# dusk-network/plonk_gadgets

Hardware: AMD Instinct MI355X
Metric: gadget constraints/sec (range_check 256-bit) (higher is better)
Workload: dtype u64x4 (BLS12-381 scalar, Montgomery limbs); 1 GPU; C2: 2^20 witnesses/GPU x (allocate + range_check(min=0,max=2^254)), n=255, 1031 rows + 1034 vars per witness; items_per_gpu=1048576, items_per_launch=1048576

## Files before the change

### plonk_gadgets_amd/csrc/capi.hip

```cpp
#include "../../include/plonk_gadgets_hip.h"

#include <hip/hip_runtime.h>

#include <algorithm>
#include <cstdio>
#include <cstdlib>
#include <cstring>
#include <initializer_list>
#include <new>
#include <functional>
#include <string>
#include <type_traits>
#include <utility>
#include <vector>

#include "emit.hpp"
#include "fr.hpp"
#include "range_gadgets.hpp"
#include "scalar_gadgets.hpp"
#include "composer.hpp"
#include "permutation.hpp"
#include "materialize.hpp"
#include "permutation_product.hpp"
#include "ntt.hpp"
// ... 63 lines not shown
}
pg_status check_u64s(const void *p, const char *what, bool nullable = false) {
    if (!p && nullable) return PG_OK;
    if (!p || !aligned(p, 8)) return fail(PG_ERR_INVALID_ARGUMENT, std::string(what) + " NULL or not 8-byte aligned");
    return PG_OK;
}

}

struct pg_engine {
    int device = -1;
    int num_cus = 0;
    uint4 *d_pow2 = nullptr;
    uint32_t *d_rows = nullptr, *d_vars = nullptr;
    uint64_t *d_blk_rows = nullptr, *d_blk_vars = nullptr;
    unsigned long long *d_blk_agg = nullptr;
    uint32_t *d_err_count = nullptr;
    uint64_t scratch_items = 0, scratch_blocks = 0;
    using PlanResult = pg::PlanTotals;
    PlanResult *h_plan = nullptr;
    uint4 *d_prefix = nullptr;
    uint64_t inv_elems = 0;
    hipStream_t side = nullptr;
    hipEvent_t ev_fork = nullptr, ev_inv = nullptr;
    hipStream_t last_stream = nullptr;
    bool have_last = false;
    hipEvent_t ev_switch = nullptr;
    uint4 *d_pp = nullptr;
    uint64_t pp_units = 0;
    uint4 *d_ntt = nullptr;
    uint64_t ntt_units = 0;
    uint4 *d_quot = nullptr, *d_eval = nullptr;
    uint64_t quot_units = 0, eval_units = 0;
};

namespace {

pg_status ensure_scratch(pg_engine *e, uint64_t batch) {
    if (batch <= e->scratch_items && e->d_err_count) return PG_OK;
    PG_HIP_TRY(hipSetDevice(e->device));
    if (e->d_rows) { (void)hipFree(e->d_rows); e->d_rows = nullptr; }
    if (e->d_vars) { (void)hipFree(e->d_vars); e->d_vars = nullptr; }
    if (e->d_blk_rows) { (void)hipFree(e->d_blk_rows); e->d_blk_rows = nullptr; }
    if (e->d_blk_vars) { (void)hipFree(e->d_blk_vars); e->d_blk_vars = nullptr; }
    if (e->d_blk_agg) { (void)hipFree(e->d_blk_agg); e->d_blk_agg = nullptr; }
    e->scratch_items = 0;
    const uint64_t items = batch < 1024 ? 1024 : batch;
    const uint64_t nblk = std::max<uint64_t>((items + pg::kScanBlock - 1) / pg::kScanBlock, 2048);
    PG_HIP_TRY(hipMalloc(&e->d_rows, items * sizeof(uint32_t)));
    PG_HIP_TRY(hipMalloc(&e->d_vars, items * sizeof(uint32_t)));
    PG_HIP_TRY(hipMalloc(&e->d_blk_rows, nblk * sizeof(uint64_t)));
    PG_HIP_TRY(hipMalloc(&e->d_blk_vars, nblk * sizeof(uint64_t)));
    PG_HIP_TRY(hipMalloc(&e->d_blk_agg, (nblk + 1) * sizeof(unsigned long long)));
    PG_HIP_TRY(hipMemset(e->d_blk_agg, 0, (nblk + 1) * sizeof(unsigned long long)));
    e->scratch_blocks = nblk;
    if (!e->d_err_count) {
        PG_HIP_TRY(hipMalloc(&e->d_err_count, sizeof(uint32_t)));
        PG_HIP_TRY(hipMemset(e->d_err_count, 0, sizeof(uint32_t)));
    }
    e->scratch_items = items;
    return PG_OK;
}

pg::PlanScan plan_scan(pg_engine *e, uint64_t batch, uint64_t *d_row_off, uint64_t *d_var_off, bool with_errs) {
    const uint64_t nblk = (batch + pg::kScanBlock - 1) / pg::kScanBlock;
    pg::PlanScan P{};
// ... 1356 lines not shown
```

### plonk_gadgets_amd/csrc/capi_composer.inc

```

struct pg_composer {
    pg_engine *e = nullptr;
    hipStream_t stream = nullptr;
    uint64_t gate_cap = 0, var_cap = 0, n = 0, nvars = 0, zero_var = 0;
    pg::ComposerCols cols{};
    uint64_t *d_stage = nullptr;
    std::vector<uint64_t> pi_gate;
    std::vector<pg_scalar> pi_val;
    std::vector<pg::FourthWire> fourth;
    std::vector<pg::PermSeg> segs;
    void *perm_small = nullptr, *perm_big = nullptr, *val_ws = nullptr;
    void *perm_pieces = nullptr;
    size_t perm_pieces_bytes = 0;
    size_t perm_small_bytes = 0, perm_big_bytes = 0, val_ws_bytes = 0;
    std::vector<void *> ragged;
    uint64_t *h_total = nullptr;
    uint64_t perm_last_sparse = 0;
    uint64_t sparse_hint = 0;
    uint64_t sparse_cap_first = 0;
    bool auto_grow = false;
    uint64_t col_stride = 0;
    void *block = nullptr;
    struct Queued {
        uint8_t kind;
        pg::GateCmd g;
        pg::Fr b0, b1;
        uint32_t num_bits;
        uint64_t wvar;
        pg::Fr wval;
        uint64_t gate, var;
        bool in_place = false;
    };
    std::vector<Queued> queue;
    bool queueing = true;
    pg_scalar last_min{}, last_max{};
    pg_layout last_lay{};
    int last_kind = 0;
    struct Staging {
        char *h = nullptr, *d = nullptr;
        size_t bytes = 0;
        hipEvent_t ev = nullptr;
    } staging[2];
    int stage = 0;
    size_t queue_used = 0;
    uint64_t flushes = 0, flush_launches = 0;
    struct Sig {
// ... 613 lines not shown
    c->rows_in_place = c->rows_rewritten = 0;
    return PG_OK;
}

pg_status pg_composer_refresh_stats(const pg_composer *c, uint64_t *rows_in_place, uint64_t *rows_rewritten, int *refreshing) {
    if (!c) return fail(PG_ERR_INVALID_ARGUMENT, "composer is NULL");
    if (rows_in_place) *rows_in_place = c->rows_in_place;
    if (rows_rewritten) *rows_rewritten = c->rows_rewritten;
    if (refreshing) *refreshing = c->refill ? 1 : 0;
    return PG_OK;
}

void pg_composer_destroy(pg_composer *c) {
    if (!c) return;
    (void)hipSetDevice(c->e->device);
    (void)hipStreamSynchronize(c->stream);
    if (c->block) {
        (void)hipFree(c->block);
    } else {
        for (int i = 0; i < 5; i++) if (c->cols.q[i]) (void)hipFree(c->cols.q[i]);
        for (int i = 0; i < 3; i++) if (c->cols.w[i]) (void)hipFree(c->cols.w[i]);
        if (c->cols.vars) (void)hipFree(c->cols.vars);
    }
    if (c->d_stage) (void)hipFree(c->d_stage);
    for (pg_composer::Staging &S : c->staging) {
        if (S.d) (void)hipFree(S.d);
        if (S.h) (void)hipHostFree(S.h);
        if (S.ev) (void)hipEventDestroy(S.ev);
    }
    if (c->perm_small) (void)hipFree(c->perm_small);
    if (c->perm_big) (void)hipFree(c->perm_big);
    if (c->val_ws) (void)hipFree(c->val_ws);
    if (c->perm_pieces) (void)hipFree(c->perm_pieces);
    for (void *p : c->ragged) (void)hipFree(p);
    if (c->h_total) (void)hipHostFree(c->h_total);
    delete c;
}

uint64_t pg_composer_circuit_size(const pg_composer *c) { return c ? c->n : 0; }
uint64_t pg_composer_num_variables(const pg_composer *c) { return c ? c->nvars : 0; }
pg_variable pg_composer_zero_var(const pg_composer *c) { return c ? c->zero_var : 0; }

pg_status pg_composer_columns(const pg_composer *c, pg_columns *out) {
    if (!c || !out) return fail(PG_ERR_INVALID_ARGUMENT, "NULL argument");
    PG_TRY(flush(const_cast<pg_composer *>(c)));
    *out = cols_at(c, 0, 0);
    return PG_OK;
}

pg_status pg_composer_reserve(pg_composer *c, uint64_t gate_capacity, uint64_t var_capacity) {
    if (!c) return fail(PG_ERR_INVALID_ARGUMENT, "composer is NULL");
    return grow(c, gate_capacity, var_capacity);
}
pg_status pg_composer_spread_columns(pg_composer *c, uint64_t stride_bytes) {
    if (!c) return fail(PG_ERR_INVALID_ARGUMENT, "composer is NULL");
    if (stride_bytes > (1ull << 44)) return fail(PG_ERR_INVALID_ARGUMENT, "stride too large");
    if (stride_bytes == c->col_stride) return PG_OK;
    const uint64_t before = c->col_stride;
    c->col_stride = stride_bytes;
    const pg_status st = grow(c, c->gate_cap, c->var_cap, true);
    if (st != PG_OK) c->col_stride = before;
    return st;
}
pg_status pg_composer_auto_grow(pg_composer *c, int on) {
    if (!c) return fail(PG_ERR_INVALID_ARGUMENT, "composer is NULL");
    c->auto_grow = on != 0;
// ... 858 lines not shown
        else if (s.wire_kind == pg::WIRES_MAX_BOUND_ALLOCATED) PG_MAT_LAUNCH(pg::MAT_SELF, pg::WIRES_MAX_BOUND_ALLOCATED);
        else if (s.wire_kind == pg::WIRES_DECOMPOSITION) PG_MAT_LAUNCH(pg::MAT_SELF, pg::WIRES_DECOMPOSITION);
        else if (s.wire_kind == pg::WIRES_MIX) PG_MAT_LAUNCH(pg::MAT_SELF, pg::WIRES_MIX);
        else PG_MAT_LAUNCH(pg::MAT_READ_WIRES, pg::WIRES_UNKNOWN);
#undef PG_MAT_LAUNCH
        at = s.gate_end;
    }
    generic(at, c->n);
    CallBuffers B(c->stream);
    uint64_t *d_gate; uint4 *d_val; pg::FourthWire *d_fw;
    PG_TRY(upload_sparse(c, B, &d_gate, &d_val, &d_fw));
    if (d_fw)
        hipLaunchKernelGGL(pg::patch_fourth_kernel, dim3(1), dim3(64), 0, c->stream, reinterpret_cast<uint4 *>(out->q_4), out->w_4,
                           reinterpret_cast<uint4 *>(out->w_4_value), c->cols.vars, d_fw, (uint32_t)c->fourth.size());
    PG_HIP_TRY(hipGetLastError());
    PG_HIP_TRY(hipStreamSynchronize(c->stream));
    return PG_OK;
}

#ifndef PG_PERM_LDS_PAD
#define PG_PERM_LDS_PAD 0
#endif
static pg_status perm_reserve(pg_composer *c, void **buf, size_t *have, size_t bytes) {
    if (bytes <= *have) return PG_OK;
    PG_HIP_TRY(hipStreamSynchronize(c->stream));
    if (*buf) (void)hipFree(*buf);
    *buf = nullptr;
    *have = 0;
    PG_HIP_TRY(hipMalloc(buf, bytes));
    *have = bytes;
    return PG_OK;
}

pg_status pg_composer_permutation_reserve(pg_composer *c, uint64_t sparse_positions) {
    if (!c) return fail(PG_ERR_INVALID_ARGUMENT, "composer is NULL");
    c->sparse_cap_first = sparse_positions;
    if (sparse_positions) c->perm_last_sparse = 0;
    return PG_OK;
}

pg_status pg_composer_permutation(pg_composer *c, uint64_t padded_n, uint64_t *d_sigma) {
    if (!c) return fail(PG_ERR_INVALID_ARGUMENT, "composer is NULL");
    PG_TRY(flush(c));
    PG_TRY(check_u64s(d_sigma, "d_sigma"));
    if (padded_n < c->n) return fail(PG_ERR_INVALID_ARGUMENT, "padded_n is smaller than the circuit");
    PG_HIP_TRY(hipSetDevice(c->e->device));
    const uint32_t grid = (uint32_t)c->e->num_cus * 32;
    if (!c->h_total) PG_HIP_TRY(hipHostMalloc(reinterpret_cast<void **>(&c->h_total), 32, hipHostMallocDefault));
    uint32_t pos_bits = 2, var_bits = 1;
    while ((1ull << pos_bits) < 4 * c->n) pos_bits++;
    while ((1ull << var_bits) < c->nvars + 1) var_bits++;
    if (pos_bits + var_bits > 64) return fail(PG_ERR_INVALID_ARGUMENT, "circuit too large for 64-bit (Variable, position) keys");
    std::vector<pg::PermSeg> segs;
    std::vector<std::pair<uint64_t, uint64_t>> gaps;
    uint64_t at = 0, gap_rows = 0;
    for (pg::PermSeg s : c->segs) {
        const auto fits = [&](uint64_t k) {
            return 4 * k * s.L < pg::kPermDone && k * s.V < pg::kPermNone &&
                   pg::perm_local_lds_bytes((uint32_t)(k * s.L), (uint32_t)(k * s.V)) <= pg::kPermLocalLdsLimit;
        };
        if (!fits(1)) continue;
        uint64_t k = 1024 / s.L;
        k = k < 1 ? 1 : (k > s.items ? s.items : k);
        while (k > 1 && !fits(k)) k--;
        const bool closed_ladder = s.wire_kind != pg::WIRES_UNKNOWN && s.wire_kind < pg::WIRES_MIX && (s.row_off ? s.wire_kind == pg::WIRES_MAX_BOUND && s.tail == 0 : s.wire_n >= 2);
        if (closed_ladder || (pg::is_template_kind(s.wire_kind) && s.tail == 0)) k = 1;
        s.group = (uint32_t)k;
        if (s.gate_base > at) gaps.emplace_back(at, s.gate_base);
        segs.push_back(s);
        at = s.gate_end;
    }
    if (c->n > at) gaps.emplace_back(at, c->n);
    for (const auto &g : gaps) gap_rows += g.second - g.first;
    const size_t seg_bytes = (segs.size() * sizeof(pg::PermSeg) + 255) / 256 * 256;
    const size_t fw_bytes = (c->fourth.size() * sizeof(pg::FourthWire) + 255) / 256 * 256;
    PG_TRY(perm_reserve(c, &c->perm_small, &c->perm_small_bytes, seg_bytes + fw_bytes + 256));
    char *small = static_cast<char *>(c->perm_small);
    pg::PermCtx X;
    X.C = c->cols; X.n = c->n; X.padded_n = padded_n; X.zero_var = c->zero_var;
    X.segs = reinterpret_cast<const pg::PermSeg *>(small); X.n_segs = (uint32_t)segs.size();
    X.fw = reinterpret_cast<const pg::FourthWire *>(small + seg_bytes); X.n_fw = (uint32_t)c->fourth.size();
    X.fw_lo = 0; X.fw_span = 0; X.pos_bits = pos_bits;
    X.hole_key = pos_bits + var_bits >= 64 ? ~0ull : (1ull << (pos_bits + var_bits)) - 1;
    if (!c->fourth.empty()) {
        uint64_t lo = ~0ull, hi = 0;
        for (const pg::FourthWire &f : c->fourth) { lo = f.gate < lo ? f.gate : lo; hi = f.gate > hi ? f.gate : hi; }
        X.fw_lo = lo; X.fw_span = hi - lo;
    }
    uint64_t reserved = 0;
    for (pg::PermSeg &s : segs)
        if (s.wire_kind != pg::WIRES_UNKNOWN && !s.row_off && s.wire_n >= 2) {
            s.sparse_base = reserved;
            reserved += s.items * pg::ladder_foreign_per_item(s.wire_kind);
        } else if (pg::is_template_kind(s.wire_kind) && s.tail == 0) {
            s.sparse_base = reserved;
            reserved += s.items * pg::template_foreign_per_item(s.wire_kind);
        }
    const auto ragged_ladder = [](const pg::PermSeg &s) { return s.row_off && s.wire_kind == pg::WIRES_MAX_BOUND && s.tail == 0; };
    const auto template_seg = [](const pg::PermSeg &s) { return pg::is_template_kind(s.wire_kind) && s.tail == 0; };
    const auto needs_pieces = [&](const pg::PermSeg &s) { return ragged_ladder(s) || (template_seg(s) && s.row_off); };
    const auto pieces_of = [](const pg::PermSeg &s) { return (s.gate_end - (s.gate_base & ~1ull) + pg::kPermLadderRows - 1) / pg::kPermLadderRows; };
    {
        uint64_t total_pieces = 0;
        for (const pg::PermSeg &s : segs)
            if (needs_pieces(s)) total_pieces += pieces_of(s);
        if (total_pieces) {
            PG_TRY(perm_reserve(c, &c->perm_pieces, &c->perm_pieces_bytes, total_pieces * sizeof(uint32_t)));
            uint32_t *at_piece = static_cast<uint32_t *>(c->perm_pieces);
            for (pg::PermSeg &s : segs)
                if (needs_pieces(s)) {
                    s.piece_item = at_piece;
                    at_piece += pieces_of(s);
                    const uint64_t want = (s.items + pg::kThreads - 1) / pg::kThreads;
                    hipLaunchKernelGGL(pg::perm_piece_items_kernel, dim3((uint32_t)(want < grid ? want : grid)), dim3(pg::kThreads), 0, c->stream, s,
                                       pg::kPermLadderRows, at_piece - pieces_of(s));
                }
            PG_HIP_TRY(hipGetLastError());
        }
    }
    unsigned long long *d_count = reinterpret_cast<unsigned long long *>(small + seg_bytes + fw_bytes);
    if (!segs.empty())
        PG_HIP_TRY(hipMemcpyAsync(small, segs.data(), segs.size() * sizeof(pg::PermSeg), hipMemcpyHostToDevice, c->stream));
    if (!c->fourth.empty())
        PG_HIP_TRY(hipMemcpyAsync(small + seg_bytes, c->fourth.data(), c->fourth.size() * sizeof(pg::FourthWire),
                                  hipMemcpyHostToDevice, c->stream));
    uint64_t cap = c->sparse_cap_first ? c->sparse_cap_first : 4 * gap_rows + c->sparse_hint + (1ull << 16), nS = 0;
    if (cap < c->perm_last_sparse) cap = c->perm_last_sparse;
    uint64_t *k0 = nullptr, *k1 = nullptr, holes = 0;
    size_t tmp_bytes = 0;
    for (int attempt = 0;; attempt++) {
        uint64_t *nul = nullptr;
        PG_HIP_TRY(rocprim::radix_sort_keys(nullptr, tmp_bytes, nul, nul, (size_t)cap, 0u, pos_bits + var_bits, c->stream));
        const size_t kb = (cap * 8 + 255) / 256 * 256;
        PG_TRY(perm_reserve(c, &c->perm_big, &c->perm_big_bytes, 2 * kb + tmp_bytes + 256));
        k0 = reinterpret_cast<uint64_t *>(c->perm_big);
        k1 = reinterpret_cast<uint64_t *>(static_cast<char *>(c->perm_big) + kb);
        const pg::PermSparse Q{k0, d_count, cap};
        hipLaunchKernelGGL(pg::perm_count_init_kernel, dim3(1), dim3(1), 0, c->stream, d_count, reserved);
        for (const pg::PermSeg &s : segs) {
            const uint64_t groups = (s.items + s.group - 1) / s.group, most = (uint64_t)c->e->num_cus * 64;
            if (s.wire_kind != pg::WIRES_UNKNOWN && !s.row_off && s.wire_n >= 2) {
                const uint64_t pieces = (s.gate_end - (s.gate_base & ~1ull) + pg::kPermLadderRows - 1) / pg::kPermLadderRows;
                const uint64_t lmost = pg::kPermLadderRows <= 2048 ? 0x7fffffffull : most;
                if (pg::kPermLadderLds)
                    PG_HIP_TRY(hipFuncSetAttribute(reinterpret_cast<const void *>(pg::perm_ladder_kernel<false>), hipFuncAttributeMaxDynamicSharedMemorySize,
                                                   (int)pg::kPermLadderLds));
                const uint32_t lds = pg::ladder_foreign_per_item(s.wire_kind) ? 0u : pg::kPermLadderLds;
                hipLaunchKernelGGL(pg::perm_ladder_kernel<false>, dim3((uint32_t)(pieces < lmost ? pieces : lmost)), dim3(pg::kThreads), lds,
                                   c->stream, X, s, Q, d_sigma);
                continue;
            }
            if (template_seg(s)) {
                const uint64_t pieces = pieces_of(s);
                if (pieces > 0x7fffffffull) return fail(PG_ERR_INVALID_ARGUMENT, "segment too large for one launch");
                const uint32_t lds = pg::template_foreign_per_item(s.wire_kind) ? 0u : pg::kPermLadderLds - 8192;
                const pg::TemplateRows T = pg::template_rows(s.wire_kind);
                if (s.row_off) {
                    PG_HIP_TRY(hipFuncSetAttribute(reinterpret_cast<const void *>(pg::perm_template_kernel<true>),
                                                   hipFuncAttributeMaxDynamicSharedMemorySize, (int)pg::kPermLadderLds));
                    hipLaunchKernelGGL(pg::perm_template_kernel<true>, dim3((uint32_t)pieces), dim3(pg::kThreads), lds, c->stream, X, s, T, Q, d_sigma);
                } else {
                    PG_HIP_TRY(hipFuncSetAttribute(reinterpret_cast<const void *>(pg::perm_template_kernel<false>),
                                                   hipFuncAttributeMaxDynamicSharedMemorySize, (int)pg::kPermLadderLds));
                    hipLaunchKernelGGL(pg::perm_template_kernel<false>, dim3((uint32_t)pieces), dim3(pg::kThreads), lds, c->stream, X, s, T, Q, d_sigma);
                }
                continue;
            }
            if (ragged_ladder(s)) {
                const uint64_t pieces = pieces_of(s);
                if (pieces > 0x7fffffffull) return fail(PG_ERR_INVALID_ARGUMENT, "segment too large for one launch");
                if (pg::kPermLadderLds)
                    PG_HIP_TRY(hipFuncSetAttribute(reinterpret_cast<const void *>(pg::perm_ladder_kernel<true>), hipFuncAttributeMaxDynamicSharedMemorySize,
                                                   (int)pg::kPermLadderLds));
                hipLaunchKernelGGL(pg::perm_ladder_kernel<true>, dim3((uint32_t)pieces), dim3(pg::kThreads), pg::kPermLadderLds, c->stream, X, s, Q,
                                   d_sigma);
                continue;
            }
            hipLaunchKernelGGL(pg::perm_item_kernel, dim3((uint32_t)(groups < most ? groups : most)), dim3(pg::kThreads),
                               pg::perm_local_lds_bytes(s.group * s.L, s.group * s.V) + PG_PERM_LDS_PAD, c->stream, X, s, groups, Q, d_sigma);
        }
        for (const auto &g : gaps) {
            const uint64_t nblk = (g.second - g.first + pg::kPermChunk - 1) / pg::kPermChunk;
            hipLaunchKernelGGL(pg::perm_gap_kernel, dim3((uint32_t)nblk), dim3(pg::kThreads), 0, c->stream, X, g.first, g.second, Q,
                               d_sigma);
        }
        PG_HIP_TRY(hipMemcpyAsync(c->h_total, d_count, 16, hipMemcpyDeviceToHost, c->stream));
        PG_HIP_TRY(hipStreamSynchronize(c->stream));
        nS = c->h_total[0];
        holes = c->h_total[1];
        c->perm_last_sparse = nS;
        if (nS <= cap) break;
        if (attempt) return fail(PG_ERR_HIP, "sparse position list grew between two passes");
        cap = nS;
    }
    if (nS) {
        PG_HIP_TRY(rocprim::radix_sort_keys(static_cast<char *>(c->perm_big) + 2 * ((cap * 8 + 255) / 256 * 256), tmp_bytes, k0, k1,
                                            (size_t)nS, 0u, pos_bits + var_bits, c->stream));
        nS -= holes;
    }
    if (nS) {
        const uint64_t want = (nS + pg::kThreads - 1) / pg::kThreads;
        hipLaunchKernelGGL(pg::perm_sparse_link_kernel, dim3((uint32_t)(want < grid ? want : grid)), dim3(pg::kThreads), 0, c->stream,
                           X, k1, nS, d_sigma);
        if (!segs.empty()) {
            const uint64_t wantw = (nS + 255) / 256;
            hipLaunchKernelGGL(pg::perm_splice_kernel, dim3((uint32_t)(wantw < grid ? wantw : grid)), dim3(pg::kThreads), 0, c->stream,
                               X, k1, nS, d_sigma);
        }
    }
    if (padded_n > c->n) {
        const uint64_t per_run = ((padded_n - c->n) / 2 + 1 + pg::kPermIdentityUnits - 1) / pg::kPermIdentityUnits;
        if (4 * per_run > 0x7fffffffull) return fail(PG_ERR_INVALID_ARGUMENT, "padding too large for one launch");
        PG_HIP_TRY(hipFuncSetAttribute(reinterpret_cast<const void *>(pg::perm_identity_kernel), hipFuncAttributeMaxDynamicSharedMemorySize,
                                       (int)pg::kPermIdentityLds));
        hipLaunchKernelGGL(pg::perm_identity_kernel, dim3((uint32_t)(4 * per_run)), dim3(pg::kThreads), pg::kPermIdentityLds, c->stream,
                           d_sigma, c->n, padded_n);
    }
    PG_HIP_TRY(hipGetLastError());
    return PG_OK;
}

pg_status pg_check_rows(pg_engine *e, const pg_columns *cols, uint64_t n_gates, uint64_t var_base, uint64_t n_vars,
                        pg_variable zero_var, int64_t *first_bad, void *stream) {
    if (!e || !first_bad) return fail(PG_ERR_INVALID_ARGUMENT, "NULL argument");
    *first_bad = -1;
    if (n_gates == 0) return PG_OK;
    PG_TRY(check_columns(cols));
    PG_HIP_TRY(hipSetDevice(e->device));
    hipStream_t st = static_cast<hipStream_t>(stream);
    pg::ComposerCols C;
    C.q[0] = reinterpret_cast<uint4 *>(cols->q_m); C.q[1] = reinterpret_cast<uint4 *>(cols->q_l);
    C.q[2] = reinterpret_cast<uint4 *>(cols->q_r); C.q[3] = reinterpret_cast<uint4 *>(cols->q_o);
    C.q[4] = reinterpret_cast<uint4 *>(cols->q_c);
    C.w[0] = cols->w_l; C.w[1] = cols->w_r; C.w[2] = cols->w_o;
    C.vars = reinterpret_cast<uint4 *>(cols->var_values);
    unsigned long long *d_bad = nullptr, h_bad = ~0ull;
    PG_HIP_TRY(hipMalloc(&d_bad, 8));
    PG_HIP_TRY(hipMemcpyAsync(d_bad, &h_bad, 8, hipMemcpyHostToDevice, st));
    hipLaunchKernelGGL(pg::check_kernel, dim3((uint32_t)e->num_cus * 16), dim3(pg::kThreads), 0, st, C, n_gates, var_base, n_vars,
                       zero_var, (const uint64_t *)nullptr, (const uint4 *)nullptr, 0u, (const pg::FourthWire *)nullptr, 0u, d_bad);
    hipError_t le = hipGetLastError();
    if (le == hipSuccess) le = hipMemcpyAsync(&h_bad, d_bad, 8, hipMemcpyDeviceToHost, st);
    if (le == hipSuccess) le = hipStreamSynchronize(st);
    (void)hipFree(d_bad);
    if (le != hipSuccess) return fail(PG_ERR_HIP, std::string("pg_check_rows: ") + hipGetErrorString(le));
    *first_bad = h_bad == ~0ull ? -1 : (int64_t)h_bad;
    return PG_OK;
// ... 4 lines not shown
```

### plonk_gadgets_amd/csrc/experiment.hpp

```cpp
#pragma once

#if !defined(PG_EXPERIMENT) &&                                                                                                  \
    (defined(PG_NT_STORES) || defined(PG_FULL_BARRIERS) || defined(PG_EMIT_WAVES_PER_SIMD) || defined(PG_XCD_REMAP) ||          \
     defined(PG_UNALIGNED_SWEEPS) || defined(PG_ROWS_WAVES_PER_SIMD) || defined(PG_ROWS_SETPRIO) || defined(PG_INVERT_FERMAT) || \
     defined(PG_INV_GRP) || defined(PG_RC_W) || defined(PG_MB_W) || defined(PG_MIX_VARS_VGPRS) || defined(PG_MIX_STAMPS) ||     \
     defined(PG_QUEUE_MAX) || defined(PG_PERM_LDS_PAD) || defined(PG_GRID_BLOCKS_PER_CU) || defined(PG_PLAN_TWO_LAUNCHES) ||    \
     defined(PG_INV_LANES_PER_CU) || defined(PG_INV_MAX_PER_LANE) || defined(PG_SIDE_STREAM_NORMAL_PRIORITY) || defined(PG_VAR_SWEEP_SINGLE) || \
     defined(PG_TILE_SPREAD) || defined(PG_MIX_EARLY_TILES) || defined(PG_MAT_THREADS) || defined(PG_MAT_UNROLL) || defined(PG_MAT_LOADS) || defined(PG_PERM_LADDER_ROWS) || defined(PG_PERM_LADDER_LDS) || defined(PG_MAT_GRID_PER_CU) || defined(PG_EMIT_GRID_BLOCKS_PER_CU))
#error "a PG_... build option is defined without -DPG_EXPERIMENT: the shipped library is built with none of them (csrc/experiment.hpp)"
#endif
```

### plonk_gadgets_amd/csrc/permutation.hpp

```cpp
#pragma once

#include <cstring>

#include <rocprim/rocprim.hpp>

#include "composer.hpp"
#include "range_gadgets.hpp"

namespace pg {

struct PermSeg {
    uint64_t gate_base, gate_end, var_base, var_end;
    uint32_t L, V;
    uint64_t items;
    const uint64_t *row_off, *var_off;
    uint32_t group;
    uint32_t wire_kind, wire_n;
    uint64_t sparse_base;
    uint32_t tail;
    const uint32_t *piece_item;
};
enum : uint32_t { WIRES_UNKNOWN = 0, WIRES_RANGE_CHECK = 1, WIRES_MAX_BOUND = 2, WIRES_RANGE_CHECK_ALLOCATED = 3, WIRES_MAX_BOUND_ALLOCATED = 4,
                  WIRES_DECOMPOSITION = 5,
                  WIRES_MIX = 6,
// ... 352 lines not shown
    }
    const uint32_t open = ladder_block_row(j, n, j2, w2);
    if (j == 0) {
        if (kind == WIRES_MAX_BOUND_ALLOCATED) return 3;
        j2[0] = 0; w2[0] = 1; j2[1] = 0; w2[1] = 0;
    } else if (open == 2) { j2[1] = 0; w2[1] = 2; }
    else if (open == 1) { j2[0] = tail ? L : 2 * n + 3; w2[0] = tail ? 0 : 2; }
    return 0;
}

__device__ __forceinline__ uint32_t ladder_foreign_wires(uint32_t kind, uint32_t n, uint32_t j) {
    if (kind == WIRES_RANGE_CHECK_ALLOCATED) return j == 0 || j == 2 * n + 5 ? 3u : 0u;
    if (kind == WIRES_MAX_BOUND_ALLOCATED) return j == 0 ? 3u : 0u;
    if (kind == WIRES_DECOMPOSITION) return j == 2 * n + 1 ? 2u : 0u;
    return 0u;
}

__host__ __device__ inline uint32_t ladder_foreign_per_item(uint32_t kind) {
    return kind == WIRES_RANGE_CHECK_ALLOCATED ? 4u : kind == WIRES_MAX_BOUND_ALLOCATED ? 2u : kind == WIRES_DECOMPOSITION ? 1u : 0u;
}
__device__ __forceinline__ uint32_t ladder_foreign_rank(uint32_t kind, uint32_t j, uint32_t w) {
    if (kind == WIRES_DECOMPOSITION) return 0u;
    return (j ? 2u : 0u) + w;
}

#ifndef PG_PERM_LADDER_ROWS
#define PG_PERM_LADDER_ROWS 512
#endif
#ifndef PG_PERM_LADDER_LDS
#define PG_PERM_LADDER_LDS 39936
#endif
constexpr uint32_t kPermLadderRows = PG_PERM_LADDER_ROWS;
constexpr uint32_t kPermLadderLds = PG_PERM_LADDER_LDS;
constexpr uint32_t kPermRaggedWindow = 64;
__global__ __launch_bounds__(kThreads) void perm_piece_items_kernel(const PermSeg S, uint32_t rows_per_piece, uint32_t *piece_item) {
    const uint64_t d = S.gate_base & 1;
    for (uint64_t i = (uint64_t)blockIdx.x * kThreads + threadIdx.x; i < S.items; i += (uint64_t)gridDim.x * kThreads) {
        const uint64_t r0 = S.row_off[i], r1 = S.row_off[i + 1];
        if (i == 0) piece_item[0] = 0;
        for (uint64_t p = (r0 + d + rows_per_piece - 1) / rows_per_piece; p * rows_per_piece < r1 + d; p++)
            if (p) piece_item[p] = (uint32_t)i;
    }
}

template <bool RAGGED>
__global__ __launch_bounds__(kThreads) void perm_ladder_kernel(const PermCtx X, const PermSeg S, const PermSparse Q, uint64_t *sigma) {
    extern __shared__ uint4 perm_ladder_pad[];
    __shared__ uint32_t s_off[RAGGED ? kPermRaggedWindow : 1];
    static_assert(!RAGGED || kPermLadderRows / 9 + 3 <= kPermRaggedWindow, "a piece's items fit the window of prefix sums");
    const uint32_t lane = threadIdx.x & 63, kind = S.wire_kind;
    uint32_t n = S.wire_n;
    if (X.padded_n == 1) perm_ladder_pad[threadIdx.x] = make_uint4(0, 0, 0, 0);
    const uint64_t first = S.gate_base & ~1ull, total = S.gate_end - first;
    const bool wide = (reinterpret_cast<uintptr_t>(sigma) & 15) == 0 && !(X.padded_n & 1);
    const uint32_t recip = (uint32_t)(((1ull << 32) + S.L - 1) / S.L);
    const bool pow2 = (X.padded_n & (X.padded_n - 1)) == 0;
    const uint32_t sh = 63u - (uint32_t)__clzll((long long)X.padded_n);
    auto enc = [&](uint64_t gate, uint32_t wire) { return pow2 ? ((uint64_t)wire << sh) + gate : perm_encode(gate, wire, X.padded_n); };
    auto zero_wires = [&](uint64_t g, uint32_t j) {
        uint32_t z = 0;
        for (uint32_t m = ladder_foreign_wires(kind, n, j); m; m &= m - 1) {
            const uint32_t w = (uint32_t)__ffs((int)m) - 1;
            if (X.C.w[w][g] == X.zero_var) z |= 1u << w;
        }
        return z;
    };
    for (uint64_t base = (uint64_t)blockIdx.x * kPermLadderRows; base < total; base += (uint64_t)gridDim.x * kPermLadderRows) {
// ... 142 lines not shown
inline TemplateRows template_rows(uint32_t kind) {
    const SegTemplate &T = kSegTemplates[kind - WIRES_MIX];
    TemplateRows R{};
    for (uint32_t sh = 0; sh < 2; sh++) {
        R.L[sh] = T.L[sh];
        R.V[sh] = T.V[sh];
        uint32_t foreign = 0;
        const uint32_t n = (uint32_t)T.L[sh] * 3;
        for (uint32_t p = 0; p < n; p++) {
            const uint8_t code = T.wire[sh][p / 3][p % 3];
            uint64_t b = 0;
            if (code < kTmplForeign) {
                uint32_t first = 0xff, next = 0xff;
                for (uint32_t q = 0; q < n; q++)
                    if (T.wire[sh][q / 3][q % 3] == code) {
                        if (first == 0xff) first = q;
                        if (q > p && next == 0xff) next = q;
                    }
                const uint32_t z = next != 0xff ? next : first;
                b = 1u | (uint64_t)code << 2 | (uint64_t)(4 * (z / 3) + z % 3) << 6;
            } else if (code < kTmplZero) {
                b = 2u | (uint64_t)foreign++ << 12;
            } else if (code == kTmplZero) {
                b = 3u;
            }
            R.row[sh][p / 3] |= b << (16 * (p % 3));
        }
        R.F[sh] = (uint8_t)foreign;
    }
    R.Fmax = (uint8_t)template_foreign_per_item(kind);
    return R;
}

constexpr uint32_t kTmplWindow = 1024;
template <bool RAGGED>
__global__ __launch_bounds__(kThreads) void perm_template_kernel(const PermCtx X, const PermSeg S, const TemplateRows T, const PermSparse Q,
                                                                uint64_t *sigma) {
    extern __shared__ uint4 perm_template_pad[];
    __shared__ uint64_t s_row[2][kTmplRows];
    __shared__ uint32_t s_off[RAGGED ? kTmplWindow : 1];
    static_assert(kPermLadderRows + 3 <= kTmplWindow, "a piece's items fit the window of prefix sums");
    if (X.padded_n == 1) perm_template_pad[threadIdx.x] = make_uint4(0, 0, 0, 0);
    const uint32_t Lf = T.L[0], Ls = T.L[1], Fmax = T.Fmax, Ff = T.F[0], Fs = T.F[1];
    if (threadIdx.x < 2 * kTmplRows) s_row[threadIdx.x / kTmplRows][threadIdx.x % kTmplRows] = T.row[threadIdx.x / kTmplRows][threadIdx.x % kTmplRows];
    __syncthreads();
    const uint64_t first = S.gate_base & ~1ull, total = S.gate_end - first;
    const bool wide = (reinterpret_cast<uintptr_t>(sigma) & 15) == 0 && !(X.padded_n & 1);
    const uint32_t recip = (uint32_t)(((1ull << 32) + Lf - 1) / Lf);
    const bool pow2 = (X.padded_n & (X.padded_n - 1)) == 0;
    const uint32_t sh_bits = 63u - (uint32_t)__clzll((long long)X.padded_n);
    auto enc = [&](uint64_t gate, uint32_t wire) { return pow2 ? ((uint64_t)wire << sh_bits) + gate : perm_encode(gate, wire, X.padded_n); };
    for (uint64_t base = (uint64_t)blockIdx.x * kPermLadderRows; base < total; base += (uint64_t)gridDim.x * kPermLadderRows) {
        const uint64_t g_first = first + base, rel = g_first < S.gate_base ? 0 : g_first - S.gate_base;
        uint64_t item0, rows0;
        if constexpr (RAGGED) {
            item0 = S.piece_item[base / kPermLadderRows];
            rows0 = S.row_off[item0];
            __syncthreads();
            for (uint32_t e = threadIdx.x; e < kTmplWindow; e += kThreads) {
                const uint64_t i = item0 + e < S.items ? item0 + e : S.items;
                s_off[e] = (uint32_t)(S.row_off[i] - rows0);
            }
            __syncthreads();
        } else {
            item0 = rel / Lf;
            rows0 = item0 * Lf;
        }
        const uint32_t j0 = (uint32_t)(rel - rows0), skip = (uint32_t)(g_first < S.gate_base ? S.gate_base - g_first : 0);
        struct Row { uint32_t item, j, sh, rows; uint64_t g_item, word; };
        auto locate = [&](uint32_t x, Row &R) {
            if constexpr (RAGGED) {
                uint32_t lo = 0;
#pragma unroll
                for (uint32_t step = kTmplWindow / 2; step; step >>= 1)
// ... 77 lines not shown
                    } else if (type == 1u) {
                        const uint32_t sc = b >> 6 & 63u;
                        out[w][h] = enc(R[h].g_item + (sc >> 2), sc & 3);
                        keep[h] |= 1u << w;
                    } else if (type == 2u) {
                        perm_sparse_put(X, Q, slot0 + (b >> 12 & 3u), X.C.w[w][g], g, w);
                    }
                }
                if (R[h].j == 0)
                    for (uint32_t k = R[h].sh ? Fs : Ff; k < Fmax; k++) {
                        if (slot0 + k < Q.cap) Q.keys[slot0 + k] = X.hole_key;
                        atomicAdd(Q.count + 1, 1ull);
                    }
                if (g + 1 < S.gate_end) out[3][h] = enc(g + 1, (uint32_t)__ffs((int)(zm[h + 1] | 8u)) - 1);
                else out[3][h] = perm_next_zero_from(X, S.gate_end);
                keep[h] |= 8u;
            }
            const uint64_t g = g_first + t;
#pragma unroll
            for (uint32_t w = 0; w < 4; w++) {
                const bool k0 = live[0] && (keep[0] >> w & 1), k1 = live[1] && (keep[1] >> w & 1);
                uint64_t *dst = sigma + enc(g, w);
                if (wide && k0 && k1)
                    store16(reinterpret_cast<uint4 *>(dst), make_uint4((uint32_t)out[w][0], (uint32_t)(out[w][0] >> 32), (uint32_t)out[w][1],
                                                                      (uint32_t)(out[w][1] >> 32)));
                else {
                    if (k0) dst[0] = out[w][0];
                    if (k1) dst[1] = out[w][1];
                }
            }
        }
    }
    (void)Ls;
}

__global__ __launch_bounds__(kThreads) void perm_sparse_link_kernel(const PermCtx X, const uint64_t *keys, uint64_t nS,
                                                                   uint64_t *sigma) {
    const uint64_t pos_mask = (1ull << X.pos_bits) - 1;
    for (uint64_t j = (uint64_t)blockIdx.x * kThreads + threadIdx.x; j < nS; j += (uint64_t)gridDim.x * kThreads) {
        const uint64_t key = keys[j], v = key >> X.pos_bits;
        uint64_t succ;
        if (j + 1 < nS && keys[j + 1] >> X.pos_bits == v) succ = keys[j + 1];
        else {
            if (perm_home_seg(X, v) >= 0) continue;
            uint64_t h = j;
            while (h > 0 && keys[h - 1] >> X.pos_bits == v) h--;
            succ = keys[h];
        }
        sigma[perm_encode_pos(key & pos_mask, X.padded_n)] = perm_encode_pos(succ & pos_mask, X.padded_n);
    }
}

__global__ __launch_bounds__(kThreads) void perm_splice_kernel(const PermCtx X, const uint64_t *keys, uint64_t nS, uint64_t *sigma) {
    const uint32_t lane = threadIdx.x & 63;
    const uint64_t pos_mask = (1ull << X.pos_bits) - 1;
    const uint64_t waves = (uint64_t)gridDim.x * (kThreads / 64);
    for (uint64_t jb = ((uint64_t)blockIdx.x * (kThreads / 64) + (threadIdx.x >> 6)) * 64; jb < nS; jb += waves * 64) {
        const uint64_t jm = jb + lane;
        int my_seg = -1;
        if (jm < nS) {
            const uint64_t vm = keys[jm] >> X.pos_bits;
            if (jm == 0 || keys[jm - 1] >> X.pos_bits != vm) my_seg = perm_home_seg(X, vm);
        }
        uint64_t hits = __ballot(my_seg >= 0);
        while (hits) {
            const uint32_t src = (uint32_t)__ffsll((long long)hits) - 1;
// ... 62 lines not shown
```

Before: 32.56 billion constraints/s.

## Add periodic-table sigma kernel for uniform range-check and template segments

Adds a periodic permutation path. Uniform ladder segments (range-check, max-bound) and foreign-free template segments get a small per-row offset table, built once per segment. A per-wire kernel then writes sigma as gate plus a table lookup, so per-item ladder logic is no longer recomputed. The repeated hipFuncSetAttribute calls per launch are also hoisted into a one-time per-engine setup. The cost is an extra table kernel and buffer, plus a new code path that must match the old ladder output exactly.

```diff
diff --git a/plonk_gadgets_amd/csrc/capi.hip b/plonk_gadgets_amd/csrc/capi.hip
--- a/plonk_gadgets_amd/csrc/capi.hip
+++ b/plonk_gadgets_amd/csrc/capi.hip
@@ -119,6 +119,7 @@
     uint64_t ntt_units = 0;
     uint4 *d_quot = nullptr, *d_eval = nullptr;
     uint64_t quot_units = 0, eval_units = 0;
+    bool perm_attributes = false;
 };
 
 namespace {
diff --git a/plonk_gadgets_amd/csrc/capi_composer.inc b/plonk_gadgets_amd/csrc/capi_composer.inc
--- a/plonk_gadgets_amd/csrc/capi_composer.inc
+++ b/plonk_gadgets_amd/csrc/capi_composer.inc
@@ -12,6 +12,8 @@
     void *perm_small = nullptr, *perm_big = nullptr, *val_ws = nullptr;
     void *perm_pieces = nullptr;
     size_t perm_pieces_bytes = 0;
+    void *perm_tables = nullptr;
+    size_t perm_tables_bytes = 0;
     size_t perm_small_bytes = 0, perm_big_bytes = 0, val_ws_bytes = 0;
     std::vector<void *> ragged;
     uint64_t *h_total = nullptr;
@@ -691,6 +693,7 @@
     if (c->perm_big) (void)hipFree(c->perm_big);
     if (c->val_ws) (void)hipFree(c->val_ws);
     if (c->perm_pieces) (void)hipFree(c->perm_pieces);
+    if (c->perm_tables) (void)hipFree(c->perm_tables);
     for (void *p : c->ragged) (void)hipFree(p);
     if (c->h_total) (void)hipHostFree(c->h_total);
     delete c;
@@ -1615,6 +1618,22 @@
     return PG_OK;
 }
 
+static pg_status perm_attributes(pg_engine *e) {
+    if (e->perm_attributes) return PG_OK;
+    const auto raise = [](const void *f, uint32_t bytes) { return hipFuncSetAttribute(f, hipFuncAttributeMaxDynamicSharedMemorySize, (int)bytes); };
+    if (pg::kPermLadderLds) {
+        PG_HIP_TRY(raise(reinterpret_cast<const void *>(pg::perm_ladder_kernel<false>), pg::kPermLadderLds));
+        PG_HIP_TRY(raise(reinterpret_cast<const void *>(pg::perm_ladder_kernel<true>), pg::kPermLadderLds));
+        PG_HIP_TRY(raise(reinterpret_cast<const void *>(pg::perm_template_kernel<false>), pg::kPermLadderLds));
+        PG_HIP_TRY(raise(reinterpret_cast<const void *>(pg::perm_template_kernel<true>), pg::kPermLadderLds));
+    }
+    PG_HIP_TRY(raise(reinterpret_cast<const void *>(pg::perm_periodic_kernel<false>), pg::kPermPeriodicLds));
+    PG_HIP_TRY(raise(reinterpret_cast<const void *>(pg::perm_periodic_kernel<true>), pg::kPermPeriodicLds));
+    PG_HIP_TRY(raise(reinterpret_cast<const void *>(pg::perm_identity_kernel), pg::kPermIdentityLds));
+    e->perm_attributes = true;
+    return PG_OK;
+}
+
 pg_status pg_composer_permutation_reserve(pg_composer *c, uint64_t sparse_positions) {
     if (!c) return fail(PG_ERR_INVALID_ARGUMENT, "composer is NULL");
     c->sparse_cap_first = sparse_positions;
@@ -1628,6 +1647,7 @@
     PG_TRY(check_u64s(d_sigma, "d_sigma"));
     if (padded_n < c->n) return fail(PG_ERR_INVALID_ARGUMENT, "padded_n is smaller than the circuit");
     PG_HIP_TRY(hipSetDevice(c->e->device));
+    PG_TRY(perm_attributes(c->e));
     const uint32_t grid = (uint32_t)c->e->num_cus * 32;
     if (!c->h_total) PG_HIP_TRY(hipHostMalloc(reinterpret_cast<void **>(&c->h_total), 32, hipHostMallocDefault));
     uint32_t pos_bits = 2, var_bits = 1;
@@ -1681,8 +1701,16 @@
         }
     const auto ragged_ladder = [](const pg::PermSeg &s) { return s.row_off && s.wire_kind == pg::WIRES_MAX_BOUND && s.tail == 0; };
     const auto template_seg = [](const pg::PermSeg &s) { return pg::is_template_kind(s.wire_kind) && s.tail == 0; };
+    const auto periodic_mode = [&](const pg::PermSeg &s) -> int {
+        const bool own_only_ladder = s.wire_kind == pg::WIRES_RANGE_CHECK || s.wire_kind == pg::WIRES_MAX_BOUND;
+        if (own_only_ladder && !s.row_off && s.wire_n >= 2 && s.L < 32768) return pg::kPeriodicUniform;
+        if (template_seg(s) && pg::template_foreign_per_item(s.wire_kind) == 0 && !s.row_off)
+            return s.L == pg::template_rows(s.wire_kind).L[0] ? pg::kPeriodicUniform : -1;
+        return -1;
+    };
     const auto needs_pieces = [&](const pg::PermSeg &s) { return ragged_ladder(s) || (template_seg(s) && s.row_off); };
-    const auto pieces_of = [](const pg::PermSeg &s) { return (s.gate_end - (s.gate_base & ~1ull) + pg::kPermLadderRows - 1) / pg::kPermLadderRows; };
+    const auto piece_rows = [&](const pg::PermSeg &s) { return periodic_mode(s) >= 0 ? pg::kPermPeriodicRows : pg::kPermLadderRows; };
+    const auto pieces_of = [&](const pg::PermSeg &s) { return (s.gate_end - (s.gate_base & ~1ull) + piece_rows(s) - 1) / piece_rows(s); };
     {
         uint64_t total_pieces = 0;
         for (const pg::PermSeg &s : segs)
@@ -1696,7 +1724,7 @@
                     at_piece += pieces_of(s);
                     const uint64_t want = (s.items + pg::kThreads - 1) / pg::kThreads;
                     hipLaunchKernelGGL(pg::perm_piece_items_kernel, dim3((uint32_t)(want < grid ? want : grid)), dim3(pg::kThreads), 0, c->stream, s,
-                                       pg::kPermLadderRows, at_piece - pieces_of(s));
+                                       piece_rows(s), at_piece - pieces_of(s));
                 }
             PG_HIP_TRY(hipGetLastError());
         }
@@ -1707,6 +1735,31 @@
     if (!c->fourth.empty())
         PG_HIP_TRY(hipMemcpyAsync(small + seg_bytes, c->fourth.data(), c->fourth.size() * sizeof(pg::FourthWire),
                                   hipMemcpyHostToDevice, c->stream));
+    std::vector<int64_t *> tables(segs.size(), nullptr);
+    {
+        size_t bytes = 0;
+        for (const pg::PermSeg &s : segs)
+            if (periodic_mode(s) >= 0) {
+                const pg::TemplateRows T = pg::is_template_kind(s.wire_kind) ? pg::template_rows(s.wire_kind) : pg::TemplateRows{};
+                bytes += (32 * pg::periodic_table_rows((uint32_t)periodic_mode(s), s.L, T.L[1]) + 255) / 256 * 256;
+            }
+        if (bytes) {
+            PG_TRY(perm_reserve(c, &c->perm_tables, &c->perm_tables_bytes, bytes));
+            char *at_table = static_cast<char *>(c->perm_tables);
+            for (size_t i = 0; i < segs.size(); i++) {
+                const pg::PermSeg &s = segs[i];
+                const int mode = periodic_mode(s);
+                if (mode < 0) continue;
+                const pg::TemplateRows T = pg::is_template_kind(s.wire_kind) ? pg::template_rows(s.wire_kind) : pg::TemplateRows{};
+                const uint64_t rows = pg::periodic_table_rows((uint32_t)mode, s.L, T.L[1]), want = (rows + pg::kThreads - 1) / pg::kThreads;
+                tables[i] = reinterpret_cast<int64_t *>(at_table);
+                at_table += (32 * rows + 255) / 256 * 256;
+                hipLaunchKernelGGL(pg::perm_periodic_table_kernel, dim3((uint32_t)(want < grid ? want : grid)), dim3(pg::kThreads), 0, c->stream,
+                                   X, s, T, (uint32_t)mode, rows, tables[i], d_sigma);
+            }
+            PG_HIP_TRY(hipGetLastError());
+        }
+    }
     uint64_t cap = c->sparse_cap_first ? c->sparse_cap_first : 4 * gap_rows + c->sparse_hint + (1ull << 16), nS = 0;
     if (cap < c->perm_last_sparse) cap = c->perm_last_sparse;
     uint64_t *k0 = nullptr, *k1 = nullptr, holes = 0;
@@ -1720,14 +1773,28 @@
         k1 = reinterpret_cast<uint64_t *>(static_cast<char *>(c->perm_big) + kb);
         const pg::PermSparse Q{k0, d_count, cap};
         hipLaunchKernelGGL(pg::perm_count_init_kernel, dim3(1), dim3(1), 0, c->stream, d_count, reserved);
-        for (const pg::PermSeg &s : segs) {
+        for (size_t si = 0; si < segs.size(); si++) {
+            const pg::PermSeg &s = segs[si];
             const uint64_t groups = (s.items + s.group - 1) / s.group, most = (uint64_t)c->e->num_cus * 64;
+            if (const int mode = periodic_mode(s); mode >= 0) {
+                const uint64_t blocks = 4 * pieces_of(s);
+                if (blocks > 0x7fffffffull) return fail(PG_ERR_INVALID_ARGUMENT, "segment too large for one launch");
+                const pg::TemplateRows T = pg::is_template_kind(s.wire_kind) ? pg::template_rows(s.wire_kind) : pg::TemplateRows{};
+                const uint64_t rows = pg::periodic_table_rows((uint32_t)mode, s.L, T.L[1]);
+                if (mode == pg::kPeriodicUniform)
+                    hipLaunchKernelGGL(pg::perm_periodic_kernel<false>, dim3((uint32_t)blocks), dim3(pg::kThreads), pg::kPermPeriodicLds, c->stream,
+                                       X, s, (uint32_t)mode, s.L, 1u, tables[si], rows, d_sigma);
+                else
+                    hipLaunchKernelGGL(pg::perm_periodic_kernel<true>, dim3((uint32_t)blocks), dim3(pg::kThreads), pg::kPermPeriodicLds, c->stream,
+                                       X, s, (uint32_t)mode, (uint32_t)(mode == pg::kPeriodicTemplateRagged ? T.L[0] : 0u),
+                                       mode == pg::kPeriodicTemplateRagged ? pg::periodic_window(T.L[1] < T.L[0] ? T.L[1] : T.L[0], T.L[0])
+                                                                           : pg::periodic_window(pg::kPeriodicLadderMinRows, s.L),
+                                       tables[si], rows, d_sigma);
+                continue;
+            }
             if (s.wire_kind != pg::WIRES_UNKNOWN && !s.row_off && s.wire_n >= 2) {
                 const uint64_t pieces = (s.gate_end - (s.gate_base & ~1ull) + pg::kPermLadderRows - 1) / pg::kPermLadderRows;
                 const uint64_t lmost = pg::kPermLadderRows <= 2048 ? 0x7fffffffull : most;
-                if (pg::kPermLadderLds)
-                    PG_HIP_TRY(hipFuncSetAttribute(reinterpret_cast<const void *>(pg::perm_ladder_kernel<false>), hipFuncAttributeMaxDynamicSharedMemorySize,
-                                                   (int)pg::kPermLadderLds));
                 const uint32_t lds = pg::ladder_foreign_per_item(s.wire_kind) ? 0u : pg::kPermLadderLds;
                 hipLaunchKernelGGL(pg::perm_ladder_kernel<false>, dim3((uint32_t)(pieces < lmost ? pieces : lmost)), dim3(pg::kThreads), lds,
                                    c->stream, X, s, Q, d_sigma);
@@ -1739,12 +1806,8 @@
                 const uint32_t lds = pg::template_foreign_per_item(s.wire_kind) ? 0u : pg::kPermLadderLds - 8192;
                 const pg::TemplateRows T = pg::template_rows(s.wire_kind);
                 if (s.row_off) {
-                    PG_HIP_TRY(hipFuncSetAttribute(reinterpret_cast<const void *>(pg::perm_template_kernel<true>),
-                                                   hipFuncAttributeMaxDynamicSharedMemorySize, (int)pg::kPermLadderLds));
                     hipLaunchKernelGGL(pg::perm_template_kernel<true>, dim3((uint32_t)pieces), dim3(pg::kThreads), lds, c->stream, X, s, T, Q, d_sigma);
                 } else {
-                    PG_HIP_TRY(hipFuncSetAttribute(reinterpret_cast<const void *>(pg::perm_template_kernel<false>),
-                                                   hipFuncAttributeMaxDynamicSharedMemorySize, (int)pg::kPermLadderLds));
                     hipLaunchKernelGGL(pg::perm_template_kernel<false>, dim3((uint32_t)pieces), dim3(pg::kThreads), lds, c->stream, X, s, T, Q, d_sigma);
                 }
                 continue;
@@ -1752,9 +1815,6 @@
             if (ragged_ladder(s)) {
                 const uint64_t pieces = pieces_of(s);
                 if (pieces > 0x7fffffffull) return fail(PG_ERR_INVALID_ARGUMENT, "segment too large for one launch");
-                if (pg::kPermLadderLds)
-                    PG_HIP_TRY(hipFuncSetAttribute(reinterpret_cast<const void *>(pg::perm_ladder_kernel<true>), hipFuncAttributeMaxDynamicSharedMemorySize,
-                                                   (int)pg::kPermLadderLds));
                 hipLaunchKernelGGL(pg::perm_ladder_kernel<true>, dim3((uint32_t)pieces), dim3(pg::kThreads), pg::kPermLadderLds, c->stream, X, s, Q,
                                    d_sigma);
                 continue;
@@ -1794,8 +1854,6 @@
     if (padded_n > c->n) {
         const uint64_t per_run = ((padded_n - c->n) / 2 + 1 + pg::kPermIdentityUnits - 1) / pg::kPermIdentityUnits;
         if (4 * per_run > 0x7fffffffull) return fail(PG_ERR_INVALID_ARGUMENT, "padding too large for one launch");
-        PG_HIP_TRY(hipFuncSetAttribute(reinterpret_cast<const void *>(pg::perm_identity_kernel), hipFuncAttributeMaxDynamicSharedMemorySize,
-                                       (int)pg::kPermIdentityLds));
         hipLaunchKernelGGL(pg::perm_identity_kernel, dim3((uint32_t)(4 * per_run)), dim3(pg::kThreads), pg::kPermIdentityLds, c->stream,
                            d_sigma, c->n, padded_n);
     }
diff --git a/plonk_gadgets_amd/csrc/experiment.hpp b/plonk_gadgets_amd/csrc/experiment.hpp
--- a/plonk_gadgets_amd/csrc/experiment.hpp
+++ b/plonk_gadgets_amd/csrc/experiment.hpp
@@ -6,6 +6,6 @@
      defined(PG_INV_GRP) || defined(PG_RC_W) || defined(PG_MB_W) || defined(PG_MIX_VARS_VGPRS) || defined(PG_MIX_STAMPS) ||     \
      defined(PG_QUEUE_MAX) || defined(PG_PERM_LDS_PAD) || defined(PG_GRID_BLOCKS_PER_CU) || defined(PG_PLAN_TWO_LAUNCHES) ||    \
      defined(PG_INV_LANES_PER_CU) || defined(PG_INV_MAX_PER_LANE) || defined(PG_SIDE_STREAM_NORMAL_PRIORITY) || defined(PG_VAR_SWEEP_SINGLE) || \
-     defined(PG_TILE_SPREAD) || defined(PG_MIX_EARLY_TILES) || defined(PG_MAT_THREADS) || defined(PG_MAT_UNROLL) || defined(PG_MAT_LOADS) || defined(PG_PERM_LADDER_ROWS) || defined(PG_PERM_LADDER_LDS) || defined(PG_MAT_GRID_PER_CU) || defined(PG_EMIT_GRID_BLOCKS_PER_CU))
+     defined(PG_TILE_SPREAD) || defined(PG_MIX_EARLY_TILES) || defined(PG_MAT_THREADS) || defined(PG_MAT_UNROLL) || defined(PG_MAT_LOADS) || defined(PG_PERM_LADDER_ROWS) || defined(PG_PERM_LADDER_LDS) || defined(PG_PERM_PERIODIC_LDS) || defined(PG_MAT_GRID_PER_CU) || defined(PG_EMIT_GRID_BLOCKS_PER_CU))
 #error "a PG_... build option is defined without -DPG_EXPERIMENT: the shipped library is built with none of them (csrc/experiment.hpp)"
 #endif
diff --git a/plonk_gadgets_amd/csrc/permutation.hpp b/plonk_gadgets_amd/csrc/permutation.hpp
--- a/plonk_gadgets_amd/csrc/permutation.hpp
+++ b/plonk_gadgets_amd/csrc/permutation.hpp
@@ -408,7 +408,8 @@
 #endif
 constexpr uint32_t kPermLadderRows = PG_PERM_LADDER_ROWS;
 constexpr uint32_t kPermLadderLds = PG_PERM_LADDER_LDS;
-constexpr uint32_t kPermRaggedWindow = 64;
+__host__ __device__ constexpr uint32_t perm_pow2_at_least(uint32_t x) { return x <= 1 ? 1u : 2u * perm_pow2_at_least((x + 1) / 2); }
+constexpr uint32_t kPermRaggedWindow = perm_pow2_at_least(kPermLadderRows / 9 + 3);
 __global__ __launch_bounds__(kThreads) void perm_piece_items_kernel(const PermSeg S, uint32_t rows_per_piece, uint32_t *piece_item) {
     const uint64_t d = S.gate_base & 1;
     for (uint64_t i = (uint64_t)blockIdx.x * kThreads + threadIdx.x; i < S.items; i += (uint64_t)gridDim.x * kThreads) {
@@ -617,14 +618,13 @@
     return R;
 }
 
-constexpr uint32_t kTmplWindow = 1024;
+constexpr uint32_t kTmplWindow = perm_pow2_at_least(kPermLadderRows + 16);
 template <bool RAGGED>
 __global__ __launch_bounds__(kThreads) void perm_template_kernel(const PermCtx X, const PermSeg S, const TemplateRows T, const PermSparse Q,
                                                                 uint64_t *sigma) {
     extern __shared__ uint4 perm_template_pad[];
     __shared__ uint64_t s_row[2][kTmplRows];
     __shared__ uint32_t s_off[RAGGED ? kTmplWindow : 1];
-    static_assert(kPermLadderRows + 3 <= kTmplWindow, "a piece's items fit the window of prefix sums");
     if (X.padded_n == 1) perm_template_pad[threadIdx.x] = make_uint4(0, 0, 0, 0);
     const uint32_t Lf = T.L[0], Ls = T.L[1], Fmax = T.Fmax, Ff = T.F[0], Fs = T.F[1];
     if (threadIdx.x < 2 * kTmplRows) s_row[threadIdx.x / kTmplRows][threadIdx.x % kTmplRows] = T.row[threadIdx.x / kTmplRows][threadIdx.x % kTmplRows];
@@ -768,6 +768,157 @@
         }
     }
     (void)Ls;
+}
+
+enum : uint32_t { kPeriodicUniform = 0, kPeriodicLadderRagged = 1, kPeriodicTemplateRagged = 2 };
+#ifndef PG_PERM_PERIODIC_LDS
+#define PG_PERM_PERIODIC_LDS 39936
+#endif
+constexpr uint32_t kPermPeriodicLds = PG_PERM_PERIODIC_LDS;
+constexpr uint32_t kPermPeriodicUnits = 2 * kThreads;
+constexpr uint32_t kPermPeriodicRows = 2 * kPermPeriodicUnits;
+constexpr uint32_t kPeriodicLadderMinRows = 9;
+constexpr uint32_t kPermPeriodicWindow = 256;
+__host__ __device__ inline uint32_t periodic_window(uint32_t L_min, uint32_t L_max) {
+    return perm_pow2_at_least((kPermPeriodicRows + L_max) / L_min + 3);
+}
+__host__ __device__ inline uint64_t periodic_table_rows(uint32_t mode, uint32_t L, uint32_t L_short) {
+    if (mode == kPeriodicLadderRagged) {
+        const uint64_t nmax = L > 2 * 256 + 5 ? (L - 5) / 2 : 256;
+        return (nmax + 1) * (nmax + 5);
+    }
+    return mode == kPeriodicTemplateRagged ? (uint64_t)L + L_short : L;
+}
+__device__ __forceinline__ uint32_t periodic_row(uint32_t mode, uint32_t L_i, uint32_t L_full, uint32_t j) {
+    if (mode == kPeriodicLadderRagged) {
+        const uint32_t n = (L_i - 5) >> 1;
+        return n * (n + 4) + j;
+    }
+    return (L_i == L_full ? 0u : L_full) + j;
+}
+__device__ __forceinline__ uint32_t template_zero_wires(uint64_t word) {
+    uint32_t z = 0;
+#pragma unroll
+    for (uint32_t w = 0; w < 3; w++)
+        if (((uint32_t)(word >> (16 * w)) & 3u) == 3u) z |= 1u << w;
+    return z;
+}
+
+__global__ __launch_bounds__(kThreads) void perm_periodic_table_kernel(const PermCtx X, const PermSeg S, const TemplateRows T, uint32_t mode,
+                                                                      uint64_t rows, int64_t *table, uint64_t *sigma) {
+    const int64_t P = (int64_t)X.padded_n;
+    const uint32_t kind = S.wire_kind;
+    for (uint64_t r = (uint64_t)blockIdx.x * kThreads + threadIdx.x; r < rows; r += (uint64_t)gridDim.x * kThreads) {
+        int64_t add[4];
+        if (is_template_kind(kind)) {
+            const uint32_t sh = mode == kPeriodicTemplateRagged && r >= T.L[0] ? 1u : 0u, j = (uint32_t)r - (sh ? T.L[0] : 0u), L = T.L[sh];
+            const uint64_t word = T.row[sh][j];
+            const uint32_t zw = template_zero_wires(word);
+#pragma unroll
+            for (uint32_t w = 0; w < 3; w++) {
+                const uint32_t b = (uint32_t)(word >> (16 * w)) & 0xffffu;
+                if ((b & 3u) == 3u) {
+                    const uint32_t later = (zw | 8u) & ~((2u << w) - 1);
+                    add[w] = (int64_t)(__ffs((int)later) - 1) * P;
+                } else {
+                    const uint32_t sc = b >> 6 & 63u;
+                    add[w] = (int64_t)(sc & 3u) * P + (int64_t)(sc >> 2) - (int64_t)j;
+                }
+            }
+            const uint64_t next = j + 1 < L ? T.row[sh][j + 1] : T.row[0][0];
+            add[3] = (int64_t)(__ffs((int)(template_zero_wires(next) | 8u)) - 1) * P + 1;
+        } else {
+            uint32_t n = S.wire_n, j = (uint32_t)r;
+            if (mode == kPeriodicLadderRagged) {
+                n = (uint32_t)sqrtf((float)r + 4.0f);
+                n = n >= 2 ? n - 2 : 0;
+                while ((uint64_t)(n + 1) * (n + 5) <= r) n++;
+                while (n && (uint64_t)n * (n + 4) > r) n--;
+                j = (uint32_t)(r - (uint64_t)n * (n + 4));
+            }
+            uint32_t j2[3], w2[3];
+            (void)ladder_row(kind, n, j, j2, w2, S.tail);
+#pragma unroll
+            for (uint32_t w = 0; w < 3; w++) add[w] = (int64_t)w2[w] * P + (int64_t)j2[w] - (int64_t)j;
+            add[3] = 3 * P + 1;
+        }
+#pragma unroll
+        for (uint32_t w = 0; w < 4; w++) table[w * rows + r] = add[w];
+    }
+    if (blockIdx.x == 0 && threadIdx.x == 0) sigma[perm_encode(S.gate_end - 1, 3, X.padded_n)] = perm_next_zero_from(X, S.gate_end);
+}
+
+template <bool RAGGED>
+__global__ __launch_bounds__(kThreads) void perm_periodic_kernel(const PermCtx X, const PermSeg S, uint32_t mode, uint32_t L_full,
+                                                                uint32_t window, const int64_t *table, uint64_t rows, uint64_t *sigma) {
+    typedef unsigned long long __attribute__((ext_vector_type(2))) u64x2;
+    extern __shared__ uint4 perm_periodic_pad[];
+    __shared__ uint32_t s_off[RAGGED ? kPermPeriodicWindow + 1 : 1];
+    const uint32_t wire = blockIdx.x & 3;
+    const uint64_t piece = blockIdx.x >> 2, first = S.gate_base & ~1ull, g_first = first + piece * kPermPeriodicRows;
+    const uint64_t end = wire == 3 ? S.gate_end - 1 : S.gate_end;
+    const uint64_t rel = g_first < S.gate_base ? 0 : g_first - S.gate_base;
+    const uint32_t skip = g_first < S.gate_base ? 1u : 0u;
+    const int64_t *tab = table + wire * rows;
+    uint64_t *col = sigma + wire * X.padded_n;
+    const bool wide = ((reinterpret_cast<uintptr_t>(sigma) | (X.padded_n << 3)) & 15) == 0;
+    uint32_t j0;
+    if constexpr (RAGGED) {
+        const uint64_t item0 = S.piece_item[piece], rows0 = S.row_off[item0];
+        for (uint32_t e = threadIdx.x; e <= kPermPeriodicWindow; e += kThreads) {
+            const uint64_t i = item0 + e < S.items ? item0 + e : S.items;
+            s_off[e] = e < window ? (uint32_t)(S.row_off[i] - rows0) : ~0u;
+        }
+        j0 = (uint32_t)(rel - rows0);
+        __syncthreads();
+    } else {
+        j0 = (uint32_t)(rel % S.L);
+    }
+    const uint32_t recip = RAGGED ? 0u : (uint32_t)(((1ull << 32) + S.L - 1) / S.L);
+    constexpr uint32_t U = kPermPeriodicUnits / kThreads;
+    int64_t a[U][2];
+    uint64_t out[U][2];
+    bool live[U][2];
+#pragma unroll
+    for (uint32_t k = 0; k < U; k++) {
+        const uint32_t t = 2 * (k * kThreads + threadIdx.x);
+        const uint64_t g = g_first + t;
+        const bool live0 = g >= S.gate_base && g < end, live1 = g + 1 < end;
+        const uint32_t x = j0 + t + (live1 ? 1u : 0u) - skip;
+        uint32_t r_last, r_prev;
+        if constexpr (RAGGED) {
+            uint32_t lo = 0;
+            for (uint32_t step = kPermPeriodicWindow / 2; step; step >>= 1)
+                if (s_off[lo + step] <= x) lo += step;
+            const uint32_t j = x - s_off[lo], Lp = lo ? s_off[lo] - s_off[lo - 1] : 1u;
+            r_last = periodic_row(mode, s_off[lo + 1] - s_off[lo], L_full, j);
+            r_prev = j ? r_last - 1 : periodic_row(mode, Lp, L_full, Lp - 1);
+        } else {
+            r_last = x - __umulhi(x, recip) * S.L;
+            r_prev = r_last ? r_last - 1 : S.L - 1;
+        }
+        live[k][0] = live0;
+        live[k][1] = live1;
+        a[k][1] = tab[live1 ? r_last : 0];
+        a[k][0] = tab[live0 ? (live1 ? r_prev : r_last) : 0];
+    }
+#pragma unroll
+    for (uint32_t k = 0; k < U; k++) {
+        const uint64_t g = g_first + 2 * (k * kThreads + threadIdx.x);
+        out[k][0] = g + (uint64_t)a[k][0];
+        out[k][1] = g + 1 + (uint64_t)a[k][1];
+        asm volatile("" : "+v"(out[k][0]), "+v"(out[k][1]));
+    }
+#pragma unroll
+    for (uint32_t k = 0; k < U; k++) {
+        const uint64_t g = g_first + 2 * (k * kThreads + threadIdx.x);
+        if (wide && live[k][0] && live[k][1]) *reinterpret_cast<u64x2 *>(col + g) = u64x2{out[k][0], out[k][1]};
+        else {
+            if (live[k][0]) col[g] = out[k][0];
+            if (live[k][1]) col[g + 1] = out[k][1];
+        }
+    }
+    if (X.padded_n == 1) perm_periodic_pad[threadIdx.x] = make_uint4(0, 0, 0, 0);
 }
 
 __global__ __launch_bounds__(kThreads) void perm_sparse_link_kernel(const PermCtx X, const uint64_t *keys, uint64_t nS,
```

Result: no change. 32.53 billion constraints/s, median of 3 (-0.1%).
